# GREAT-WHU/DBA-Fusion

Hardware: AMD Instinct MI355X
Metric: DBA iterations/sec (25-KF, 96-edge, 512x512) [dba_update/s] (higher is better)
Workload: dtype f32 (BA, f64 reduced system) / f16 (correlation)

## Files before the change

dba-fusion_amd/csrc/ba_host.hip:

```cpp
#include <hip/hip_runtime.h>

#include <algorithm>
#include <atomic>
#include <cstdio>
#include <cstdlib>
#include <cstring>
#include <mutex>
#include <unordered_map>
#include <vector>

#include "ba_kernels.h"

#ifndef GRAM_F32_DEFAULT
#define GRAM_F32_DEFAULT true
#endif

namespace dba {

static thread_local char g_last_error[512] = "";

void set_last_error(const char *what, hipError_t e) {
  snprintf(g_last_error, sizeof(g_last_error), "%s -> %s", what, hipGetErrorString(e));
}

// ... 2 lines not shown
  static int num(const char *name) { const char *e = getenv(name); return e ? atoi(e) : 0; }
  static bool is(const char *name, const char *prefix) { const char *e = getenv(name); return e && !strncmp(e, prefix, strlen(prefix)); }
  int deterministic = is("DBA_DETERMINISTIC", "1");
  int solve_check = is("DBA_SOLVE_CHECK", "1");
  int schur_form = is("DBA_SCHUR_KERNEL", "r") ? 1 : (is("DBA_SCHUR_KERNEL", "f") || is("DBA_SCHUR_KERNEL", "g")) ? 2 : 0;
  int lin_ppl = num("DBA_LINEARIZE_PPL");
  bool lin_no_mfma = is("DBA_LINEARIZE_MFMA", "0");
  int lin_ew = num("DBA_LIN_EW");
  bool h_full = is("DBA_H_FULL", "1");
  int schur_nch = num("DBA_SCHUR_NCH");
  int gram_threads = num("DBA_SCHUR_WAVES") == 4 ? 256 : 512;
  bool gram_f32 = getenv("DBA_SCHUR_MFMA") ? is("DBA_SCHUR_MFMA", "f3") : GRAM_F32_DEFAULT;
  bool fuse_update = !is("DBA_BA_FUSE_UPDATE", "0");
  bool stage0_fold = getenv("DBA_BA_STAGE0") ? is("DBA_BA_STAGE0", "fold") : STAGE0_FOLD_DEFAULT;
  int schur_sparse_legacy = is("DBA_SCHUR_SPARSE", "legacy");
};
static const BaEnv &ba_env() { static const BaEnv env; return env; }

static std::atomic<int> g_schur_form{ba_env().schur_form};
static std::atomic<int> g_deterministic{ba_env().deterministic};
static std::atomic<int> g_solve_check{ba_env().solve_check};
static std::atomic<int> g_schur_sparse_legacy{ba_env().schur_sparse_legacy};

__global__ __launch_bounds__(256) void ba_solve_check_kernel(const double *__restrict__ H, const double *__restrict__ b, int n, double lm,
                                                             double ep, float *__restrict__ dx, int *__restrict__ meta) {
  __shared__ double s_res[256], s_mag[256];
  __shared__ int s_bad;
  if (meta[1] != 0) return;
  double res = 0.0, mag = 0.0;
  for (int i = threadIdx.x; i < n; i += blockDim.x) {
    double acc = -b[i], m = fabs(b[i]);
    for (int j = 0; j < n; j++) {
      double h = H[(size_t)max(i, j) * n + min(i, j)];
      if (i == j) h = fma(lm, h, h) + ep;
      const double t = h * (double)dx[j];
      acc += t, m += fabs(t);
    }
// ... 69 lines not shown
  L.E = take(sizeof(float) * (size_t)(P + N) * 6 * HW);
  L.Q = take(sizeof(float) * (size_t)Mmax * HW);
  L.w = take(sizeof(float) * (size_t)Mmax * HW);
  const size_t o_hparte = take(sizeof(float) * (size_t)(N > 0 ? N : 1) * nparts_max * HPE_STRIDE);
  const size_t o_aedge = take(sizeof(double) * 36 * (size_t)(N > 0 ? N : 1));
  L.dx = take(sizeof(float) * (size_t)(n6 > 0 ? n6 : 1));
  const size_t o_ptmp = take(sizeof(float) * 2 * 7 * (size_t)B);
  L.H = take(sizeof(double) * (size_t)(n6 > 0 ? n6 * (size_t)n6 : 1));
  L.b = take(sizeof(double) * (size_t)(n6 > 0 ? n6 : 1));
  size_t o_lscratch = 0;
  const bool lds_fits = ba_solve_fits_lds(n6);
  const bool want_scratch = !lds_fits || (ba_solve_band_supported(n6) && n6 >= 96);
  if (want_scratch) o_lscratch = take(sizeof(double) * ba_solve_scratch_doubles(n6));
  const size_t pairs_cap = (size_t)(P + N) * SCHUR_KP;
  const size_t o_pairs = take(sizeof(int) * 4 * (1 + pairs_cap));
  L.P = P;
  L.Mmax = Mmax;
  L.nchunks = nchunks;
  plan->layout = L;
  plan->bytes = off;
  plan->pairs_off = o_pairs, plan->pairs_cap = (int)pairs_cap;
  plan->P = P;
  plan->N = N;
  plan->B = B;
  plan->HW = HW;
  plan->nchunks = nchunks;
  plan->ht = ht, plan->wd = wd, plan->t0 = t0, plan->t1 = t1;
  if (ws) {
    if (ws_bytes < off) return DBA_ERR_WORKSPACE;
    char *base = static_cast<char *>(ws);
    plan->T.meta = reinterpret_cast<int *>(base + L.meta);
    plan->T.kx = reinterpret_cast<int *>(base + L.kx);
    plan->T.frame_slot = reinterpret_cast<int *>(base + o_fslot);
    plan->T.eoff = reinterpret_cast<int *>(base + o_eoff);
    plan->T.elist = reinterpret_cast<int *>(base + o_elist);
    plan->T.elist_rank = reinterpret_cast<int *>(base + o_erank);
    plan->T.fpose = reinterpret_cast<int *>(base + o_fpose);
    plan->T.einfo = reinterpret_cast<int *>(base + o_einfo);
    plan->T.rowinfo = reinterpret_cast<int *>(base + o_rowinfo);
    plan->T.fhead = reinterpret_cast<int *>(base + o_fhead);
    plan->T.frow = reinterpret_cast<int *>(base + o_frow);
    plan->T.gkey = reinterpret_cast<int *>(base + o_gkey);
    plan->T.pairs = reinterpret_cast<int *>(base + o_pairs);
    plan->T.pairs_cap = (int)pairs_cap;
    plan->T.Mmax = Mmax;
    plan->T.B = B;
    plan->W.E = reinterpret_cast<float *>(base + L.E);
    plan->W.Q = reinterpret_cast<float *>(base + L.Q);
    plan->W.w = reinterpret_cast<float *>(base + L.w);
    plan->W.HpartE = reinterpret_cast<float *>(base + o_hparte);
    plan->W.Aedge = reinterpret_cast<double *>(base + o_aedge);
    plan->W.dx = reinterpret_cast<float *>(base + L.dx);
    plan->W.poses_tmp = reinterpret_cast<float *>(base + o_ptmp);
    plan->W.H = reinterpret_cast<double *>(base + L.H);
    plan->W.b = reinterpret_cast<double *>(base + L.b);
    plan->W.Lscratch = want_scratch ? reinterpret_cast<double *>(base + o_lscratch) : nullptr;
    plan->W.nparts = nparts;
    plan->W.ppl = ppl;
  }
  return DBA_OK;
}

static int ba_prepare_stage(const BaPlan &plan, const int64_t *ii, const int64_t *jj, int eta_rows, int check, bool judge_band,
                            hipStream_t stream) {
  const int N = plan.N, B = plan.B, P = plan.P;
  if (N > 0 && (!ii || !jj)) return DBA_ERR_ARG;
  const int want = std::max(std::max(N, B), P);
  const int threads = std::min(1024, std::max(64, (want + 63) / 64 * 64));
  const size_t scan_ints = std::max<size_t>(std::max(threads, P), N > threads ? 1024 : 0) + 32;
  const size_t lds = sizeof(int) * ((size_t)B + 2 * (size_t)plan.T.Mmax + 1 + scan_ints + 2 * ((size_t)plan.T.Mmax + 1));
  if (lds > 160 * 1024 || P > 16384) return DBA_ERR_UNSUPPORTED;
  if (lds > 64 * 1024) {
    DBA_HIP_CHECK(hipFuncSetAttribute(reinterpret_cast<const void *>(&ba_prepare_kernel),
// ... 3 lines not shown
  int *band_verdict = max_nt ? solver_verdict_slot(plan.T.meta) : nullptr;
  hipLaunchKernelGGL(ba_prepare_kernel, dim3(1), dim3(threads), lds, stream, ii, jj, N, B, plan.t0, plan.t1,
                     (int)scan_ints, ba_schur_frame_form(N, P) ? 1 : 0, check ? 1 : 0, eta_rows,
                     eta_rows > 1 ? ws_eta_status(plan.T.meta) : nullptr, plan.T, band_verdict, max_nt);
  DBA_LAUNCH_CHECK();
  return DBA_OK;
}

static int ba_linearize_stage(const BaPlan &plan, const BaProblem &g, const float *poses, const float *disps, float alpha,
                              int upd, float *poses_out, float *disps_w, hipStream_t stream, const BaStage0 *s0 = nullptr) {
  if (!poses || !disps || !g.intrinsics || !g.disps_sens || !g.eta || g.eta_rows < 1) return DBA_ERR_ARG;
  if (g.eta_rows > 1 && g.eta_rows > plan.T.Mmax) return DBA_ERR_ARG;
  if (plan.N > 0 && (!g.targets || !g.weights || !g.jj)) return DBA_ERR_ARG;
  if (s0 && (upd != 0 || plan.W.ppl != 1)) return DBA_ERR_ARG;
  const BaStage0 none = {nullptr, 0, 0, nullptr, nullptr, 0};
#define LAUNCH_LIN_TF(PPL, MF, EW, TF)                                                                                        \
  hipLaunchKernelGGL((ba_linearize_kernel<PPL, MF, EW, TF>), dim3(plan.nchunks * EW, plan.T.Mmax + (TF ? 2 : 1)), dim3(256), 0, \
                     stream, poses, disps, g.intrinsics, g.disps_sens, g.targets, g.weights, g.eta, g.eta_rows, g.jj,         \
                     g.frame_owned, plan.N, plan.HW, plan.wd, plan.t0, plan.P, alpha, upd, poses_out, disps_w, plan.T, plan.W, \
                     TF ? *s0 : none)
#define LAUNCH_LIN(PPL, MF, EW) do { if (s0) LAUNCH_LIN_TF(PPL, MF, EW, true); else LAUNCH_LIN_TF(PPL, MF, EW, false); } while (0)
  if (plan.W.ppl == 4) LAUNCH_LIN_TF(4, false, 1, false);
  else if (plan.W.ppl == 2) LAUNCH_LIN_TF(2, false, 1, false);
  else if (ba_env().lin_no_mfma) LAUNCH_LIN(1, false, 1);
  else {
    const int env_ew = ba_env().lin_ew;
    const long waves2 = (long)plan.nchunks * 2 * 4 * plan.T.Mmax;
    const bool one = env_ew ? env_ew == 1 : waves2 > 4096;
    if (one) LAUNCH_LIN(1, true, 1);
    else LAUNCH_LIN(1, true, 2);
  }
#undef LAUNCH_LIN
#undef LAUNCH_LIN_TF
  DBA_LAUNCH_CHECK();
// ... 2 lines not shown

static int ba_reduce_stage(const BaPlan &plan, const int64_t *ii, const int64_t *jj, const uint8_t *frame_owned, int motion_only,
                           int lower, hipStream_t stream) {
  const int N = plan.N;
  const int ablocks = (N + 3) / 4;
  if (plan.P <= 0) return DBA_OK;
  if (ba_env().h_full) lower = 0;
  const bool fixed = g_deterministic.load(std::memory_order_relaxed) != 0;
  if (fixed) lower |= 2;
  if (!motion_only) {
    if (!ba_schur_frame_form(N, plan.P)) {
      if (g_schur_sparse_legacy.load(std::memory_order_relaxed))
        hipLaunchKernelGGL(ba_schur_kernel, dim3(plan.P + N + ablocks, SCHUR_KP, SCHUR_CH), dim3(256), 0, stream, ii, jj,
                           frame_owned, N, plan.HW, plan.t0, plan.P, lower, plan.T, plan.W);
      else
        hipLaunchKernelGGL(ba_schur_pairs_kernel, dim3(ablocks + plan.pairs_cap * SCHUR_CH), dim3(256), 0, stream, ii, jj,
                           frame_owned, N, plan.HW, plan.t0, plan.P, lower, plan.T, plan.W);
    } else {
      const int px = 1024;
      int nch = ba_env().schur_nch > 0 ? ba_env().schur_nch : (plan.HW + px - 1) / px;
      nch = std::max(1, std::min(nch, (plan.HW + 15) / 16));
      const dim3 grid((unsigned)(plan.T.Mmax * nch + ablocks));
      const int gram_threads = ba_env().gram_threads;
      const bool f32 = ba_env().gram_f32;
#define GRAM_LAUNCH(V, F)                                                                                     \
  hipLaunchKernelGGL((ba_schur_gram_kernel<V, F>), grid, dim3(gram_threads), 0, stream, ii, jj, frame_owned, \
                     N, plan.HW, plan.t0, plan.P, nch, lower, plan.T, plan.W)
      if (plan.HW % 4 == 0) { if (f32) GRAM_LAUNCH(true, true); else GRAM_LAUNCH(true, false); }
      else { if (f32) GRAM_LAUNCH(false, true); else GRAM_LAUNCH(false, false); }
#undef GRAM_LAUNCH
    }
    DBA_LAUNCH_CHECK();
  } else if (ablocks > 0) {
    hipLaunchKernelGGL(ba_assemble_kernel, dim3(ablocks), dim3(256), 0, stream, ii, jj, frame_owned, N, plan.t0, plan.P,
                       lower, plan.T, plan.W);
    DBA_LAUNCH_CHECK();
  }
// ... 20 lines not shown
  DBA_LAUNCH_CHECK();
  return DBA_OK;
}

static int ba_solve_stage(const BaPlan &plan, float lm, float ep, const int *fpose, int hint, hipStream_t stream) {
  const int rc = launch_ba_solve(plan.W.H, plan.W.b, fpose, 6 * plan.P, (double)lm, (double)ep, plan.W.dx, plan.T.meta,
                                 plan.W.Lscratch, stream, nullptr, hint, (fpose && fpose == plan.T.fpose) ? plan.T.meta + 16 : nullptr);
  if (rc != DBA_OK) return rc;
  if (g_solve_check.load(std::memory_order_relaxed)) return ba_solve_check_launch(plan, lm, ep, stream);
  return DBA_OK;
}

static int ba_update_launch(const BaPlan &plan, float *poses, float *disps, const int64_t *jj, const uint8_t *frame_owned,
                            int update_poses, int update_disps, float *dz_out, float *dx_out, hipStream_t stream,
                            const float *poses_src = nullptr, float disp_floor = 0.f) {
  dim3 grid((plan.HW + 255) / 256, plan.T.Mmax + 1 + (disp_floor > 0.f ? plan.B : 0));
  hipLaunchKernelGGL(ba_update_kernel, grid, dim3(256), 0, stream, poses, poses_src, disps, jj, frame_owned, plan.HW, plan.t0,
                     plan.P, update_poses, update_disps, dz_out, dx_out, plan.T, plan.W, disp_floor);
  DBA_LAUNCH_CHECK();
  return DBA_OK;
}

static bool ba_stage0_folds(const BaPlan &plan, const BaProblem &g, const BaRun &run) {
  return ba_env().stage0_fold && run.prepared == 2 && run.iterations > 0 && !g.frame_owned && !run.exchange && !run.window_fpose &&
         plan.W.ppl == 1 && plan.N <= FOLD_MAX_N && plan.B <= FOLD_MAX_B && (plan.N == 0 || (g.ii && g.jj));
}

int ba_run_loop(const BaPlan &plan, const BaProblem &g, float *poses, float *disps, const BaRun &run, hipStream_t stream) {
  const int *fpose = run.window_fpose ? run.window_fpose : plan.T.fpose;
  int rc;
  const bool fold = ba_stage0_folds(plan, g, run);
// ... 137 lines not shown
  const int rc = ba_plan(N, B, ht, wd, t0, t1, nullptr, 0, &plan);
  if (rc != DBA_OK) return rc;
  *out = plan.layout;
  return DBA_OK;
}

int dba_ba_pairs_table(int N, int B, int ht, int wd, int t0, int t1, size_t *offset, int *capacity) {
  BaPlan plan;
  const int rc = ba_plan(N, B, ht, wd, t0, t1, nullptr, 0, &plan);
  if (rc != DBA_OK) return rc;
  if (offset) *offset = plan.pairs_off;
  if (capacity) *capacity = plan.pairs_cap;
  return DBA_OK;
}

int dba_ba_schur_sparse_select(int legacy) {
  if (legacy != 0 && legacy != 1) return DBA_ERR_ARG;
  g_schur_sparse_legacy.store(legacy, std::memory_order_relaxed);
  return DBA_OK;
}

int dba_ba_poll_eta_error(int *eta_rows, int *num_kx) { return ws_poll_eta(nullptr, eta_rows, num_kx); }

int dba_ba_poll_eta_error_ws(int N, int B, int ht, int wd, int t0, int t1, void *ws, size_t ws_bytes, int *eta_rows, int *num_kx) {
  DBA_PLAN_OR_RETURN(plan);
  return ws_poll_eta(plan.T.meta, eta_rows, num_kx);
}

int dba_ba_gather_edges(const float *target_inac, const float *weight_inac, const int64_t *ii_inac, const int64_t *jj_inac,
                        int n_inac, const int64_t *sel, int n_sel, const float *target_act, const float *weight_act,
// ... 307 lines not shown
```

dba-fusion_amd/csrc/ba_kernels.h:

```cpp
#pragma once
#include "common.h"

namespace dba {

constexpr int HPE_STRIDE = 32;
#ifndef SCHUR_KP_CFG
#define SCHUR_KP_CFG 8
#endif
#ifndef SCHUR_CH_CFG
#define SCHUR_CH_CFG 2
#endif
constexpr int SCHUR_KP = SCHUR_KP_CFG;
constexpr int SCHUR_CH = SCHUR_CH_CFG;

struct BaTables {
  int *meta;
  int *kx;
  int *frame_slot;
  int *eoff;
  int *elist;
  int *elist_rank;
  int *fpose;
  int *einfo;
  int *rowinfo;
  int *fhead;
  int *frow;
  int *gkey;
  int *pairs;
  int pairs_cap;
  int Mmax, B;
};

struct BaBuffers {
  float *E;
  float *Q;
  float *w;
  float *HpartE;
  double *Aedge;
  double *H;
  double *b;
  float *dx;
  double *Lscratch;
  float *poses_tmp;
  int nparts;
  int ppl;
};

struct BaPlan {
  BaTables T;
  BaBuffers W;
  dba_ba_layout layout;
  size_t bytes;
  size_t pairs_off;
  int pairs_cap;
  int P, N, B, HW, nchunks;
  int ht, wd, t0, t1;
};

int ba_plan(int N, int B, int ht, int wd, int t0, int t1, void *ws, size_t ws_bytes, BaPlan *plan);
#define DBA_PLAN_OR_RETURN(plan) \
  BaPlan plan;                   \
  if (const int plan_rc_ = ::dba::ba_plan(N, B, ht, wd, t0, t1, ws, ws_bytes, &plan)) return plan_rc_

constexpr int GKEY_MAGIC = 0x6b657935;
__global__ void ba_prepare_kernel(const int64_t *ii, const int64_t *jj, int N, int B, int t0, int t1, int scan_ints,
                                  int ftable, int check, int eta_rows, int *status, BaTables T, int *band_verdict, int max_nt);
bool ba_schur_frame_form(int N, int P);
struct BaStage0 {
// ... 3 lines not shown
  int max_nt;
};
constexpr int FOLD_MAX_N = 256, FOLD_MAX_B = 512;
constexpr int FOLD_SCAN_INTS = FOLD_MAX_B + 32;
template <int PPL, bool MF, int EW, bool TF>
__global__ void ba_linearize_kernel(const float *poses, const float *disps, const float *intrinsics,
                                    const float *disps_sens, const float *targets, const float *weights,
                                    const float *eta, int eta_rows, const int64_t *jj,
                                    const uint8_t *frame_owned, int N, int HW, int wd, int t0, int P,
                                    float alpha, int upd, float *poses_out, float *disps_w, BaTables T, BaBuffers W,
                                    BaStage0 S0);
__global__ void ba_assemble_kernel(const int64_t *ii, const int64_t *jj, const uint8_t *frame_owned, int N,
                                   int t0, int P, int lower, BaTables T, BaBuffers W);
__global__ void ba_schur_kernel(const int64_t *ii, const int64_t *jj, const uint8_t *frame_owned, int N, int HW,
                                int t0, int P, int lower, BaTables T, BaBuffers W);
__global__ void ba_schur_pairs_kernel(const int64_t *ii, const int64_t *jj, const uint8_t *frame_owned, int N, int HW,
                                      int t0, int P, int lower, BaTables T, BaBuffers W);
__global__ void ba_symmetrize_kernel(double *H, int n);
struct ExportArg {
  double A[36];
};
__global__ void ba_export_kernel(const double *H, const double *b, int n, double *out, int gtsam, ExportArg arg, double stab,
                                 unsigned *counter, int *host_flag, int seq);
__global__ void ba_fixed_to_f64_kernel(double *H, double *b, int n);
constexpr int GRAM_LIST_CAP = 1024;
template <bool VEC, bool F32>
__global__ void ba_schur_gram_kernel(const int64_t *ii, const int64_t *jj, const uint8_t *frame_owned, int N, int HW,
                                     int t0, int P, int nch, int lower, BaTables T, BaBuffers W);
__global__ void ba_update_kernel(float *poses, const float *poses_src, float *disps, const int64_t *jj, const uint8_t *frame_owned,
                                 int HW, int t0, int P, int update_poses, int update_disps, float *dz_out,
// ... 52 lines not shown
```

dba-fusion_amd/csrc/ba_kernels.hip:

```cpp
#include "ba_kernels.h"
#include "ba_solve_admit.h"

#include <cstdio>
#include <cstring>

namespace dba {

__device__ __forceinline__ int wave_incl_scan(int v, int lane) {
#pragma unroll
  for (int off = 1; off < 64; off <<= 1) {
    const int o = __shfl_up(v, off, 64);
    if (lane >= off) v += o;
  }
  return v;
}

__device__ void ba_prepare_body(int *sm, const int64_t *__restrict__ ii, const int64_t *__restrict__ jj, int N, int B, int t0,
                                int t1, int scan_ints, int ftable, int check, int eta_rows, int *__restrict__ status,
                                const BaTables &T, int *__restrict__ band_verdict, int max_nt) {
  int *flag = sm;
  int *cnt = sm + B;
  int *kxs = cnt + T.Mmax + 1;
  int *scan = kxs + T.Mmax;
  int *vcnt = scan + scan_ints;
// ... 127 lines not shown
          const int x = sii[q];
          const bool same = ((x & (VBIT - 1)) == f);
          rank += same;
          vrank += same ? (x >> 30) : 0;
        }
        pos = cnt[m] + rank;
        T.elist[pos] = tid;
        if (myvalid) atomicAdd(&vcnt[m], 1);
      }
      emit_edge(tid, m, pos, my_j);
    }
    if (!ftable) {
      for (int m = tid; m < T.Mmax; m += nt) T.fhead[4 * m] = -1, T.fhead[4 * m + 2] = 0;
      __syncthreads();
      if (wave == 0) {
        int carry = 0;
        for (int base = 0; base <= T.Mmax; base += 64) {
          const int m = base + lane;
          const int v = (m < T.Mmax) ? vcnt[m] : 0;
          const int pc = v * (v + 1) / 2;
          const int w = wave_incl_scan(pc, lane);
          if (m <= T.Mmax) poff[m] = carry + w - pc;
          carry += __shfl(w, 63, 64);
        }
      }
      __syncthreads();
      const int npairs = poff[T.Mmax];
      const bool listed = npairs <= T.pairs_cap;
      int4 *pl = reinterpret_cast<int4 *>(T.pairs) + 1;
      if (tid == 0) *reinterpret_cast<int4 *>(T.pairs) = make_int4(listed ? npairs : -1, 0, 0, 0);
      if (listed && myvalid) {
        const int m = slot_of(my_i), v = vcnt[m], pp = kxs[m] - t0, tg = my_j - t0;
        const int vr = ((pp >= 0 && pp < P) ? 1 : 0) + vrank;
        int o = poff[m] + vr * v - vr * (vr - 1) / 2;
        pl[o++] = make_int4(P + tid, P + tid, tg | (tg << 16), m);
        const int f = my_i & (VBIT - 1);
        for (int q = tid + 1; q < N; q++)
          if (sii[q] == (f | VBIT)) pl[o++] = make_int4(P + tid, P + q, tg | (((int)jj[q] - t0) << 16), m);
      }
// ... 364 lines not shown
    const float *__restrict__ weights, const float *__restrict__ eta, int eta_rows,
    const int64_t *__restrict__ jj, const uint8_t *__restrict__ frame_owned, int N, int HW, int wd,
    int t0, int P, float alpha, int upd_arg, float *__restrict__ poses_out, float *__restrict__ disps_w, BaTables T,
    BaBuffers W, BaStage0 S0) {
  const int upd = TF ? 0 : (T.gkey[7] ? 0 : upd_arg);
#ifdef LIN_PROF
  unsigned long long lp_ = wall_clock64();
  const unsigned long long lp_start_ = lp_;
#endif
  constexpr int EB = 16;
  __shared__ float s_pose[EB][12];
  __shared__ __attribute__((aligned(16))) float s_adj[EB][28];
  __shared__ int s_edge[EB][2];
  constexpr int RED_FLOATS = MF ? MFS_FLOATS : 64 * RED_PITCH;
  __shared__ __attribute__((aligned(16))) float s_red[4][RED_FLOATS];
  const int m = blockIdx.y;
  if constexpr (TF) {
    if (m == T.Mmax + 1) {
      static_assert(!TF || 5 * FOLD_MAX_B + 3 + FOLD_SCAN_INTS <= 4 * RED_FLOATS, "stage 0 does not fit the staging tiles");
      if (blockIdx.x == 0)
        ba_prepare_body(reinterpret_cast<int *>(&s_red[0][0]), S0.ii, jj, N, T.B, t0, S0.t1, FOLD_SCAN_INTS, S0.ftable, 1, eta_rows,
                        S0.status, T, S0.band_verdict, S0.max_nt);
      return;
    }
  }
  if (m == T.Mmax) {
    const int n6 = 6 * P;
    const size_t total = (size_t)n6 * n6;
    for (size_t i = (size_t)blockIdx.x * blockDim.x + threadIdx.x; i < total; i += (size_t)gridDim.x * blockDim.x)
      W.H[i] = 0.0;
    if (blockIdx.x == 0) {
      for (int i = threadIdx.x; i < n6; i += blockDim.x) W.b[i] = 0.0;
      if (upd && poses_out)
        for (int f = threadIdx.x; f < T.B; f += blockDim.x) {
          float pr[7];
          load_pose(poses, W.dx, f, t0, P, true, pr);
#pragma unroll
          for (int c = 0; c < 7; c++) poses_out[7 * f + c] = pr[c];
        }
    }
    return;
  }
  int frame, e0 = 0, e1 = 0;
  __shared__ int2 s_out[TF ? FOLD_MAX_N : 1];
  if constexpr (TF) {
    __shared__ unsigned s_fmask[FOLD_MAX_B / 32];
// ... 31 lines not shown
    for (int w = 0; w < 4; w++) {
      const int c = s_wcnt[w];
      before += (w < (tid >> 6)) ? c : 0;
      e1 += c;
    }
    if (mine) s_out[before + __popcll(bal & ((1ull << (tid & 63)) - 1ull))] = make_int2(tid, my_j);
  } else {
    const int M = T.meta[0];
    if (m >= M) return;
    frame = T.kx[m];
    if (frame_owned && !frame_owned[frame]) return;
  }

  const int lane = lane_id();
  const int wv = threadIdx.x >> 6, ew = wv % EW;
  const int wave_global = blockIdx.x * (4 / EW) + wv / EW;
  const int kbase = wave_global * (WAVE * PPL) + lane;
  const int nparts = W.nparts;

  float intr[4] = {intrinsics[0], intrinsics[1], intrinsics[2], intrinsics[3]};
  int kc[PPL];
  bool active[PPL];
  float u[PPL], v[PPL], disp[PPL];
#pragma unroll
  for (int q = 0; q < PPL; q++) {
    const int k = kbase + WAVE * q;
    active[q] = k < HW;
    kc[q] = active[q] ? k : 0;
    u[q] = (float)(kc[q] % wd);
    v[q] = (float)(kc[q] / wd);
    disp[q] = disps[(size_t)frame * HW + kc[q]];
// ... 24 lines not shown
  for (int batch = e0; batch < e1; batch += EB) {
    const int cnt = min(EB, e1 - batch);
    __syncthreads();
    LP(1);
    if ((int)threadIdx.x < cnt) {
      const int2 ei = TF ? s_out[batch + threadIdx.x] : *reinterpret_cast<const int2 *>(T.einfo + 2 * (batch + threadIdx.x));
      const int n = ei.x, jx = ei.y;
      double t64[3], R64[9];
      edge_pose64(poses, W.dx, frame, jx, t0, P, upd != 0, t64, R64);
      s_edge[threadIdx.x][0] = n;
      s_edge[threadIdx.x][1] = jx;
#pragma unroll
      for (int c = 0; c < 3; c++) s_pose[threadIdx.x][c] = (float)t64[c];
#pragma unroll
      for (int c = 0; c < 9; c++) s_pose[threadIdx.x][3 + c] = (float)R64[c];
      double *Aw = (blockIdx.x == 0) ? W.Aedge + (size_t)n * 36 : nullptr;
      float *As = s_adj[threadIdx.x];
#pragma unroll
      for (int k = 0; k < 3; k++) {
#pragma unroll
        for (int c = 0; c < 3; c++) {
          const double rkc = -R64[3 * k + c];
          const int k1 = (k + 1) % 3, k2 = (k + 2) % 3;
          const double x = t64[k2] * R64[3 * k1 + c] - t64[k1] * R64[3 * k2 + c];
          As[6 * k + c] = (float)rkc, As[6 * k + 3 + c] = (float)x, As[18 + 3 * k + c] = (float)rkc;
          if (Aw) Aw[6 * k + c] = rkc, Aw[6 * k + 3 + c] = x, Aw[6 * (3 + k) + c] = 0.0, Aw[6 * (3 + k) + 3 + c] = rkc;
        }
      }
    }
    __syncthreads();
    LP(2);
// ... 547 lines not shown
}

__global__ __launch_bounds__(256) void ba_schur_pairs_kernel(const int64_t *__restrict__ ii,
                                                             const int64_t *__restrict__ jj,
                                                             const uint8_t *__restrict__ frame_owned, int N, int HW,
                                                             int t0, int P, int lower, BaTables T, BaBuffers W) {
  __shared__ float red[4][44];
  const int ablk = (N + 3) / 4;
  if ((int)blockIdx.x < ablk) {
    ba_assemble_block((int)blockIdx.x, ii, jj, frame_owned, N, t0, P, lower, T, W);
    return;
  }
  const int wg = (int)blockIdx.x - ablk;
  const int np = T.pairs[0];
  if (np < 0) {
    schur_rows_body(red, wg / (SCHUR_KP * SCHUR_CH), (wg / SCHUR_CH) % SCHUR_KP, SCHUR_KP, wg % SCHUR_CH, SCHUR_CH, frame_owned,
                    HW, t0, P, lower, T, W);
    return;
  }
  const int pi = wg / SCHUR_CH, ch = wg % SCHUR_CH;
  if (pi >= np) return;
  const int4 pr = reinterpret_cast<const int4 *>(T.pairs)[1 + pi];
  const int r1 = pr.x, r2 = pr.y, tgt1 = pr.z & 0xffff, tgt2 = pr.z >> 16, m = pr.w;
  if (frame_owned && !frame_owned[T.kx[m]]) return;
  const int chunk = (HW + SCHUR_CH - 1) / SCHUR_CH;
  const int k0 = ch * chunk, k1 = min(HW, k0 + chunk);
  const bool batch = chunk <= 256 * SCHUR_BATCH;
  const float *E1 = W.E + (size_t)r1 * 6 * HW;
  const float *E2 = W.E + (size_t)r2 * 6 * HW;
  const float *Qm = W.Q + (size_t)m * HW;
  const float *wm = W.w + (size_t)m * HW;
  const int n6 = 6 * P;
  if (r1 != r2) schur_pair_block<false, false>(red, batch, E1, E2, Qm, wm, HW, k0, k1, tgt1, tgt2, n6, lower, W);
  else if (lower & 1) schur_pair_block<true, true>(red, batch, E1, E2, Qm, wm, HW, k0, k1, tgt1, tgt2, n6, lower, W);
  else schur_pair_block<true, false>(red, batch, E1, E2, Qm, wm, HW, k0, k1, tgt1, tgt2, n6, lower, W);
}

constexpr int GRAM_MAX_T = 5;
constexpr int GRAM_MAX_ROWS = (16 * GRAM_MAX_T - 1) / 6;
constexpr int GRAM_MAX_TILES = GRAM_MAX_T * (GRAM_MAX_T + 1) / 2;
typedef double gram_d4 __attribute__((ext_vector_type(4)));

template <int T>
struct GramStage {
  lin_f4 q;
  lin_f4 e[T];
};

template <int T, bool VEC>
__device__ __forceinline__ void gram_load(GramStage<T> &S, const float *const (&bp)[T], const float *qm, int g, int gend,
// ... 187 lines not shown
  }
}

template <bool VEC, bool F32>
__global__ __launch_bounds__(512, 2) void ba_schur_gram_kernel(const int64_t *__restrict__ ii, const int64_t *__restrict__ jj,
                                                               const uint8_t *__restrict__ frame_owned, int N, int HW,
                                                               int t0, int P, int nch, int lower, BaTables T, BaBuffers W) {
  __shared__ double red[GRAM_MAX_TILES * 256];
  __shared__ int s_tgt[64];
  const int tid = threadIdx.x, lane = tid & 63;
  const int ablk = (N + 3) / 4;
  if ((int)blockIdx.x < ablk) {
    if (tid < 256) ba_assemble_block((int)blockIdx.x, ii, jj, frame_owned, N, t0, P, lower, T, W);
    return;
  }
  const int fblk = (int)blockIdx.x - ablk;
  const int m = fblk / nch, ch = fblk - m * nch;
  const int4 fh = *reinterpret_cast<const int4 *>(T.fhead + 4 * m);
  const int frame = fh.x, nrows = fh.z;
  if (frame < 0 || nrows == 0) return;
  if (frame_owned && !frame_owned[frame]) return;
  const int cpx = ((HW + nch - 1) / nch + 15) / 16 * 16;
  const int c0 = ch * cpx, c1 = min(HW, c0 + cpx);
  if (c0 >= c1) return;
  const float *wm = W.w + (size_t)m * HW, *qm = W.Q + (size_t)m * HW;
  const int n6 = 6 * P;
  const int *frow = T.frow + 2 * fh.y;
  if (nrows > GRAM_MAX_ROWS) {
    gram_frame_pairs(W, wm, qm, frow, nrows, c0, c1, HW, n6, (lower & 1) != 0, (lower & 2) != 0, reinterpret_cast<float *>(red));
    return;
  }
  int my_row = 0, my_tgt = 0;
// ... 108 lines not shown
      *counter = 0;
      __threadfence_system();
      __hip_atomic_store(host_flag, seq, __ATOMIC_RELEASE, __HIP_MEMORY_SCOPE_SYSTEM);
    }
  }
}

__global__ __launch_bounds__(256) void ba_update_kernel(float *__restrict__ poses, const float *__restrict__ poses_src,
                                                        float *__restrict__ disps,
                                                        const int64_t *__restrict__ jj,
                                                        const uint8_t *__restrict__ frame_owned, int HW,
                                                        int t0, int P, int update_poses, int update_disps,
                                                        float *__restrict__ dz_out,
                                                        float *__restrict__ dx_out, BaTables T, BaBuffers W,
                                                        float disp_floor) {
  const int m = blockIdx.y;
  if (T.gkey[7]) {
    if (m == T.Mmax && blockIdx.x == 0 && dx_out)
      for (int i = threadIdx.x; i < 6 * P; i += blockDim.x) dx_out[i] = 0.f;
    const int k = blockIdx.x * blockDim.x + threadIdx.x;
    if (m < T.Mmax && k < HW && dz_out && update_disps) dz_out[(size_t)m * HW + k] = 0.f;
    return;
  }
  if (m > T.Mmax) {
    const int frame = m - T.Mmax - 1;
    const int slot = T.frame_slot[frame];
    if (update_disps && slot >= 0 && slot < T.meta[0] && (!frame_owned || frame_owned[frame])) return;
    const int k = blockIdx.x * blockDim.x + threadIdx.x;
    if (k >= HW) return;
    const size_t fk = (size_t)frame * HW + k;
    if (disps[fk] < disp_floor) disps[fk] = disp_floor;
    return;
  }
  if (m == T.Mmax) {
    if (blockIdx.x != 0) return;
    if (dx_out)
      for (int i = threadIdx.x; i < 6 * P; i += blockDim.x) dx_out[i] = W.dx[i];
    if (!update_poses) return;
    for (int p = threadIdx.x; p < P; p += blockDim.x) {
      float pr[7];
      load_pose(poses_src ? poses_src : poses, W.dx, t0 + p, t0, P, true, pr);
#pragma unroll
      for (int c = 0; c < 7; c++) poses[7 * (t0 + p) + c] = pr[c];
    }
    return;
  }
  if (!update_disps) return;
  const int M = T.meta[0];
  if (m >= M) return;
  const int frame = T.kx[m];
  if (frame_owned && !frame_owned[frame]) return;
  const int k = blockIdx.x * blockDim.x + threadIdx.x;
  if (k >= HW) return;

  const float dz = backsub_pixel(T, W, m, frame, k, HW, t0, P);
  const size_t mk = (size_t)m * HW + k;
  const size_t fk = (size_t)frame * HW + k;
  float d = disps[fk] + dz;
  if (disp_floor > 0.f) d = (d < disp_floor) ? disp_floor : d;
  disps[fk] = d;
  if (dz_out) dz_out[mk] = dz;
}

__global__ __launch_bounds__(256) void ba_gather_edges_kernel(const float2 *__restrict__ tgt_inac, const float2 *__restrict__ wgt_inac,
                                                              const int64_t *__restrict__ ii_inac, const int64_t *__restrict__ jj_inac,
                                                              const int64_t *__restrict__ sel, int n_sel, int n_inac,
                                                              const float2 *__restrict__ tgt_act, const float2 *__restrict__ wgt_act,
// ... 29 lines not shown
```

dba-fusion_amd/dbaf_amd/_lib.py:

```python
import ctypes
import os
import weakref

import torch

_HERE = os.path.dirname(os.path.abspath(__file__))
LIB_PATH = os.environ.get("DBA_HIP_LIB") or os.path.join(os.path.dirname(_HERE), "lib", "libdba_hip.so")

DBA_F32, DBA_F16, DBA_F64, DBA_U8 = 0, 1, 2, 3
_ERR = {-1: "DBA_ERR_ARG", -2: "DBA_ERR_WORKSPACE", -3: "DBA_ERR_HIP", -4: "DBA_ERR_UNSUPPORTED"}

c_int, c_float, c_size_t, c_void_p = ctypes.c_int, ctypes.c_float, ctypes.c_size_t, ctypes.c_void_p


class BaLayout(ctypes.Structure):
    _fields_ = [(n, c_size_t) for n in ("H", "b", "dx", "meta", "E", "Q", "w", "kx")] + \
               [("P", c_int), ("Mmax", c_int), ("nchunks", c_int)]


class ShardExchange(ctypes.Structure):
    _fields_ = [("world", c_int), ("rank", c_int), ("comm", c_void_p), ("peer_regions", c_void_p),
                ("peer_epoch", ctypes.POINTER(ctypes.c_uint)), ("peer_max_doubles", c_size_t), ("peer_status", c_void_p),
                ("band_idx", c_void_p), ("band_len", c_size_t), ("band_buf", c_void_p),
                ("my_rows", c_void_p), ("n_mine", c_int), ("kmax", c_int), ("all_rows", c_void_p), ("all_slots", c_void_p),
# ... 40 lines not shown
    "dba_ba_prepare_keyed": (c_int, [_P, _P] + [c_int] * 8 + [_P, c_size_t, _P]),
    "dba_ba_workspace_init": (c_int, [c_int] * 6 + [_P, c_size_t, _P]),
    "dba_ba_solver_verdict": (c_int, [c_int] * 6 + [_P, c_size_t]),
    "dba_ba_poll_eta_error": (c_int, [ctypes.POINTER(c_int), ctypes.POINTER(c_int)]),
    "dba_ba_poll_eta_error_ws": (c_int, [c_int] * 6 + [_P, c_size_t, ctypes.POINTER(c_int), ctypes.POINTER(c_int)]),
    "dba_ba_gather_edges": (c_int, [_P] * 4 + [c_int, _P, c_int] + [_P] * 4 + [c_int] * 3 + [_P] * 5),
    "dba_ba_linearize": (c_int, [_P] * 7 + [c_int] + [_P] * 3 + [c_int] * 6 + [c_float, _P, c_size_t, _P]),
    "dba_ba_reduce": (c_int, [_P] * 3 + [c_int] * 7 + [_P, c_size_t, _P]),
    "dba_ba_schur_select": (c_int, [c_int]),
    "dba_ba_schur_select_thread": (c_int, [c_int]),
    "dba_ba_schur_auto_form": (c_int, [c_int, c_int]),
    "dba_ba_schur_thread_form": (c_int, []),
    "dba_ba_schur_generation": (c_int, []),
    "dba_ba_schur_sparse_select": (c_int, [c_int]),
    "dba_ba_pairs_table": (c_int, [c_int] * 6 + [ctypes.POINTER(c_size_t), ctypes.POINTER(c_int)]),
    "dba_ba_set_deterministic": (c_int, [c_int]),
    "dba_ba_set_solve_check": (c_int, [c_int]),
    "dba_ba_solve_check": (c_int, [c_int] * 6 + [c_float, c_float, _P, c_size_t, _P]),
    "dba_ba_symmetrize": (c_int, [c_int] * 6 + [_P, c_size_t, _P]),
    "dba_ba_solve": (c_int, [c_int] * 6 + [c_float, c_float, _P, c_size_t, _P]),
    "dba_ba_solve_skyline": (c_int, [c_int] * 6 + [c_float, c_float, _P, _P, c_size_t, _P]),
    "dba_ba_update": (c_int, [_P] * 5 + [c_int] * 8 + [_P, _P, c_size_t, _P]),
    "dba_ba_shard_front": (c_int, [_P] * 7 + [c_int] + [_P] * 3 + [c_int] * 6 + [c_float, c_int, _P, c_size_t, _P]),
    "dba_ba_shard_back": (c_int, [_P] * 5 + [c_int] * 6 + [c_float, c_float, c_int, _P, c_int, _P, c_size_t, _P]),
    "dba_comm_unique_id": (c_int, [_P]),
    "dba_comm_create": (c_int, [_P, c_int, c_int, ctypes.POINTER(_P)]),
    "dba_comm_destroy": (c_int, [_P]),
    "dba_comm_info": (c_int, [_P, ctypes.POINTER(c_int), ctypes.POINTER(c_int)]),
    "dba_comm_allreduce_f64": (c_int, [_P, c_size_t, _P]),
    "dba_ba_sharded_run": (c_int, [_P] * 7 + [c_int] + [_P] * 3 + [c_int] * 7 + [c_float, c_float, c_float, c_int, _P, c_int,
# ... 229 lines not shown
```

include/dba_hip.h:

```cpp
#ifndef DBA_HIP_H
#define DBA_HIP_H

#include <stddef.h>
#include <stdint.h>

#ifdef __cplusplus
extern "C" {
#endif

enum {
  DBA_OK = 0,
  DBA_ERR_ARG = -1,
  DBA_ERR_WORKSPACE = -2,
  DBA_ERR_HIP = -3,
  DBA_ERR_UNSUPPORTED = -4
};

enum { DBA_F32 = 0, DBA_F16 = 1, DBA_F64 = 2, DBA_U8 = 3 };

typedef void *dba_stream_t;

const char *dba_version(void);
const char *dba_last_error(void);

// ... 25 lines not shown
                     const float *eta, int eta_rows, const int64_t *ii, const int64_t *jj,
                     const uint8_t *frame_owned, int N, int B, int ht, int wd, int t0, int t1,
                     float alpha, void *ws, size_t ws_bytes, dba_stream_t stream);

int dba_ba_reduce(const int64_t *ii, const int64_t *jj, const uint8_t *frame_owned, int N, int B,
                  int ht, int wd, int t0, int t1, int motion_only, void *ws, size_t ws_bytes,
                  dba_stream_t stream);

int dba_ba_schur_select(int form);
int dba_ba_schur_select_thread(int form);
int dba_ba_schur_thread_form(void);
int dba_ba_schur_auto_form(int N, int P);
int dba_ba_schur_generation(void);
int dba_ba_schur_sparse_select(int legacy);
int dba_ba_pairs_table(int N, int B, int ht, int wd, int t0, int t1, size_t *offset, int *capacity);

int dba_ba_set_deterministic(int on);

int dba_ba_set_solve_check(int on);
int dba_ba_solve_check(int N, int B, int ht, int wd, int t0, int t1, float lm, float ep, void *ws, size_t ws_bytes,
                       dba_stream_t stream);

int dba_ba_symmetrize(int N, int B, int ht, int wd, int t0, int t1, void *ws, size_t ws_bytes, dba_stream_t stream);

int dba_ba_solve(int N, int B, int ht, int wd, int t0, int t1, float lm, float ep, void *ws,
                 size_t ws_bytes, dba_stream_t stream);
int dba_ba_solve_skyline(int N, int B, int ht, int wd, int t0, int t1, float lm, float ep, const int32_t *fpose, void *ws,
                         size_t ws_bytes, dba_stream_t stream);

int dba_ba_update(float *poses, float *disps, const int64_t *ii, const int64_t *jj,
// ... 464 lines not shown
```

Measured before the change: 4124.

## Place BA linearize and Schur pair blocks on XCDs by frame for L2 locality

Adds an XCD-aware block-id remapping so that every workgroup touching a given frame (linearize) or a given frame's pair group (Schur pairs) lands on the same XCD, since consecutive block ids round-robin across the MI355X's 8 XCDs. The prepare kernel now orders the pair prefix-scan by XCD group and records per-XCD group offsets, and the Schur pairs kernel loops over several pairs per block within its XCD group. The aim is better reuse of per-frame E/Q/w data in each XCD's private L2. The cost is possible load imbalance across XCDs, extra serialized work per block, padded grids, and reliance on an assumed round-robin dispatch order. Gram and update placement are added but off by default.

```diff
diff --git a/dba-fusion_amd/csrc/ba_host.hip b/dba-fusion_amd/csrc/ba_host.hip
--- a/dba-fusion_amd/csrc/ba_host.hip
+++ b/dba-fusion_amd/csrc/ba_host.hip
@@ -40,6 +40,7 @@
   bool fuse_update = !is("DBA_BA_FUSE_UPDATE", "0");
   bool stage0_fold = getenv("DBA_BA_STAGE0") ? is("DBA_BA_STAGE0", "fold") : STAGE0_FOLD_DEFAULT;
   int schur_sparse_legacy = is("DBA_SCHUR_SPARSE", "legacy");
+  int xcd = getenv("DBA_BA_XCD") ? (num("DBA_BA_XCD") & BA_XCD_ALL) : BA_XCD_DEFAULT;
 };
 static const BaEnv &ba_env() { static const BaEnv env; return env; }
 
@@ -47,6 +48,7 @@
 static std::atomic<int> g_deterministic{ba_env().deterministic};
 static std::atomic<int> g_solve_check{ba_env().solve_check};
 static std::atomic<int> g_schur_sparse_legacy{ba_env().schur_sparse_legacy};
+static std::atomic<int> g_xcd{ba_env().xcd};
 
 __global__ __launch_bounds__(256) void ba_solve_check_kernel(const double *__restrict__ H, const double *__restrict__ b, int n, double lm,
                                                              double ep, float *__restrict__ dx, int *__restrict__ meta) {
@@ -146,12 +148,13 @@
   if (want_scratch) o_lscratch = take(sizeof(double) * ba_solve_scratch_doubles(n6));
   const size_t pairs_cap = (size_t)(P + N) * SCHUR_KP;
   const size_t o_pairs = take(sizeof(int) * 4 * (1 + pairs_cap));
+  const size_t o_pgrp = take(sizeof(int) * (BA_NUM_XCD + 1));
   L.P = P;
   L.Mmax = Mmax;
   L.nchunks = nchunks;
   plan->layout = L;
   plan->bytes = off;
-  plan->pairs_off = o_pairs, plan->pairs_cap = (int)pairs_cap;
+  plan->pairs_off = o_pairs, plan->pairs_cap = (int)pairs_cap, plan->pgrp_off = o_pgrp;
   plan->P = P;
   plan->N = N;
   plan->B = B;
@@ -175,6 +178,7 @@
     plan->T.gkey = reinterpret_cast<int *>(base + o_gkey);
     plan->T.pairs = reinterpret_cast<int *>(base + o_pairs);
     plan->T.pairs_cap = (int)pairs_cap;
+    plan->T.pgrp = reinterpret_cast<int *>(base + o_pgrp);
     plan->T.Mmax = Mmax;
     plan->T.B = B;
     plan->W.E = reinterpret_cast<float *>(base + L.E);
@@ -189,6 +193,7 @@
     plan->W.Lscratch = want_scratch ? reinterpret_cast<double *>(base + o_lscratch) : nullptr;
     plan->W.nparts = nparts;
     plan->W.ppl = ppl;
+    plan->W.xcd = g_xcd.load(std::memory_order_relaxed);
   }
   return DBA_OK;
 }
@@ -222,10 +227,17 @@
   if (plan.N > 0 && (!g.targets || !g.weights || !g.jj)) return DBA_ERR_ARG;
   if (s0 && (upd != 0 || plan.W.ppl != 1)) return DBA_ERR_ARG;
   const BaStage0 none = {nullptr, 0, 0, nullptr, nullptr, 0};
+  BaBuffers Wl = plan.W;
+  const bool placed = (plan.W.xcd & ((upd & 2) ? BA_XCD_LIN : BA_XCD_LIN_FIRST)) != 0;
+  Wl.xcd = placed ? (Wl.xcd | BA_XCD_LIN) : (Wl.xcd & ~BA_XCD_LIN);
+  auto lin_grid = [&](int chunks, int rows_behind) {
+    return placed ? dim3((unsigned)(ba_xcd_frame_ids(plan.T.Mmax, chunks) + rows_behind * chunks))
+                                     : dim3((unsigned)chunks, (unsigned)(plan.T.Mmax + rows_behind));
+  };
 #define LAUNCH_LIN_TF(PPL, MF, EW, TF)                                                                                        \
-  hipLaunchKernelGGL((ba_linearize_kernel<PPL, MF, EW, TF>), dim3(plan.nchunks * EW, plan.T.Mmax + (TF ? 2 : 1)), dim3(256), 0, \
+  hipLaunchKernelGGL((ba_linearize_kernel<PPL, MF, EW, TF>), lin_grid(plan.nchunks * EW, TF ? 2 : 1), dim3(256), 0,             \
                      stream, poses, disps, g.intrinsics, g.disps_sens, g.targets, g.weights, g.eta, g.eta_rows, g.jj,         \
-                     g.frame_owned, plan.N, plan.HW, plan.wd, plan.t0, plan.P, alpha, upd, poses_out, disps_w, plan.T, plan.W, \
+                     g.frame_owned, plan.N, plan.HW, plan.wd, plan.t0, plan.P, alpha, upd, poses_out, disps_w, plan.T, Wl,     \
                      TF ? *s0 : none)
 #define LAUNCH_LIN(PPL, MF, EW) do { if (s0) LAUNCH_LIN_TF(PPL, MF, EW, true); else LAUNCH_LIN_TF(PPL, MF, EW, false); } while (0)
   if (plan.W.ppl == 4) LAUNCH_LIN_TF(4, false, 1, false);
@@ -258,13 +270,16 @@
         hipLaunchKernelGGL(ba_schur_kernel, dim3(plan.P + N + ablocks, SCHUR_KP, SCHUR_CH), dim3(256), 0, stream, ii, jj,
                            frame_owned, N, plan.HW, plan.t0, plan.P, lower, plan.T, plan.W);
       else
-        hipLaunchKernelGGL(ba_schur_pairs_kernel, dim3(ablocks + plan.pairs_cap * SCHUR_CH), dim3(256), 0, stream, ii, jj,
-                           frame_owned, N, plan.HW, plan.t0, plan.P, lower, plan.T, plan.W);
+        hipLaunchKernelGGL(ba_schur_pairs_kernel,
+                           dim3((plan.W.xcd & BA_XCD_SCHUR) ? ba_schur_pairs_xcd_grid(N, plan.pairs_cap).ids()
+                                                            : ablocks + plan.pairs_cap * SCHUR_CH),
+                           dim3(256), 0, stream, ii, jj, frame_owned, N, plan.HW, plan.t0, plan.P, lower, plan.T, plan.W);
     } else {
       const int px = 1024;
       int nch = ba_env().schur_nch > 0 ? ba_env().schur_nch : (plan.HW + px - 1) / px;
       nch = std::max(1, std::min(nch, (plan.HW + 15) / 16));
-      const dim3 grid((unsigned)(plan.T.Mmax * nch + ablocks));
+      const dim3 grid((plan.W.xcd & BA_XCD_GRAM) ? (unsigned)(ba_xcd_round_up(ablocks) + ba_xcd_frame_ids(plan.T.Mmax, nch))
+                                                  : (unsigned)(plan.T.Mmax * nch + ablocks));
       const int gram_threads = ba_env().gram_threads;
       const bool f32 = ba_env().gram_f32;
 #define GRAM_LAUNCH(V, F)                                                                                     \
@@ -315,7 +330,9 @@
 static int ba_update_launch(const BaPlan &plan, float *poses, float *disps, const int64_t *jj, const uint8_t *frame_owned,
                             int update_poses, int update_disps, float *dz_out, float *dx_out, hipStream_t stream,
                             const float *poses_src = nullptr, float disp_floor = 0.f) {
-  dim3 grid((plan.HW + 255) / 256, plan.T.Mmax + 1 + (disp_floor > 0.f ? plan.B : 0));
+  const int chunks = (plan.HW + 255) / 256, rows_behind = 1 + (disp_floor > 0.f ? plan.B : 0);
+  dim3 grid(chunks, plan.T.Mmax + rows_behind);
+  if (plan.W.xcd & BA_XCD_UPDATE) grid = dim3((unsigned)(ba_xcd_frame_ids(plan.T.Mmax, chunks) + rows_behind * chunks));
   hipLaunchKernelGGL(ba_update_kernel, grid, dim3(256), 0, stream, poses, poses_src, disps, jj, frame_owned, plan.HW, plan.t0,
                      plan.P, update_poses, update_disps, dz_out, dx_out, plan.T, plan.W, disp_floor);
   DBA_LAUNCH_CHECK();
@@ -483,6 +500,37 @@
   return DBA_OK;
 }
 
+int dba_ba_xcd_select(int mask) {
+  if (mask < -1 || mask > BA_XCD_ALL) return DBA_ERR_ARG;
+  g_xcd.store(mask < 0 ? ba_env().xcd : mask, std::memory_order_relaxed);
+  return DBA_OK;
+}
+
+int dba_ba_xcd_mask(void) { return g_xcd.load(std::memory_order_relaxed); }
+
+int dba_ba_xcd_frame_ids(int F, int C) { return (F < 0 || C <= 0) ? DBA_ERR_ARG : ba_xcd_frame_ids(F, C); }
+
+int dba_ba_xcd_frame_item(int id, int base, int F, int C, int *item, int *row) {
+  if (F < 0 || C <= 0 || base % BA_NUM_XCD || !item || !row) return DBA_ERR_ARG;
+  return ba_xcd_frame_item(id, base, F, C, *item, *row) ? 1 : 0;
+}
+
+int dba_ba_xcd_group_item(int id, int base, int S, const int32_t *goff, int CH, int k, int *entry, int *chunk) {
+  if (S < 0 || CH <= 0 || k < 0 || base % BA_NUM_XCD || !goff || !entry || !chunk) return DBA_ERR_ARG;
+  return ba_xcd_group_item(id, base, S, goff, CH, k, *entry, *chunk) ? 1 : 0;
+}
+
+int dba_ba_xcd_pairs_grid(int N, int B, int ht, int wd, int t0, int t1, int *base, int *slots, size_t *pgrp_offset) {
+  BaPlan plan;
+  const int rc = ba_plan(N, B, ht, wd, t0, t1, nullptr, 0, &plan);
+  if (rc != DBA_OK) return rc;
+  const BaPairsXcdGrid grid = ba_schur_pairs_xcd_grid(N, plan.pairs_cap);
+  if (base) *base = grid.base;
+  if (slots) *slots = grid.S;
+  if (pgrp_offset) *pgrp_offset = plan.pgrp_off;
+  return DBA_OK;
+}
+
 int dba_ba_schur_sparse_select(int legacy) {
   if (legacy != 0 && legacy != 1) return DBA_ERR_ARG;
   g_schur_sparse_legacy.store(legacy, std::memory_order_relaxed);
diff --git a/dba-fusion_amd/csrc/ba_kernels.h b/dba-fusion_amd/csrc/ba_kernels.h
--- a/dba-fusion_amd/csrc/ba_kernels.h
+++ b/dba-fusion_amd/csrc/ba_kernels.h
@@ -1,5 +1,6 @@
 #pragma once
 #include "common.h"
+#include "ba_xcd.h"
 
 namespace dba {
 
@@ -28,6 +29,7 @@
   int *gkey;
   int *pairs;
   int pairs_cap;
+  int *pgrp;
   int Mmax, B;
 };
 
@@ -44,6 +46,7 @@
   float *poses_tmp;
   int nparts;
   int ppl;
+  int xcd;
 };
 
 struct BaPlan {
@@ -52,6 +55,7 @@
   dba_ba_layout layout;
   size_t bytes;
   size_t pairs_off;
+  size_t pgrp_off;
   int pairs_cap;
   int P, N, B, HW, nchunks;
   int ht, wd, t0, t1;
@@ -85,6 +89,13 @@
                                    int t0, int P, int lower, BaTables T, BaBuffers W);
 __global__ void ba_schur_kernel(const int64_t *ii, const int64_t *jj, const uint8_t *frame_owned, int N, int HW,
                                 int t0, int P, int lower, BaTables T, BaBuffers W);
+struct BaPairsXcdGrid {
+  int base, S;
+  int ids() const { return base + BA_NUM_XCD * S; }
+};
+inline BaPairsXcdGrid ba_schur_pairs_xcd_grid(int N, int pairs_cap) {
+  return {ba_xcd_round_up((N + 3) / 4), (pairs_cap * SCHUR_CH + BA_NUM_XCD - 1) / BA_NUM_XCD};
+}
 __global__ void ba_schur_pairs_kernel(const int64_t *ii, const int64_t *jj, const uint8_t *frame_owned, int N, int HW,
                                       int t0, int P, int lower, BaTables T, BaBuffers W);
 __global__ void ba_symmetrize_kernel(double *H, int n);
diff --git a/dba-fusion_amd/csrc/ba_kernels.hip b/dba-fusion_amd/csrc/ba_kernels.hip
--- a/dba-fusion_amd/csrc/ba_kernels.hip
+++ b/dba-fusion_amd/csrc/ba_kernels.hip
@@ -165,15 +165,21 @@
       for (int m = tid; m < T.Mmax; m += nt) T.fhead[4 * m] = -1, T.fhead[4 * m + 2] = 0;
       __syncthreads();
       if (wave == 0) {
+        const int G = (T.Mmax + BA_NUM_XCD - 1) / BA_NUM_XCD;
         int carry = 0;
-        for (int base = 0; base <= T.Mmax; base += 64) {
-          const int m = base + lane;
-          const int v = (m < T.Mmax) ? vcnt[m] : 0;
+        for (int base = 0; base < BA_NUM_XCD * G; base += 64) {
+          const int j = base + lane;
+          const int x = j / G, m = x + BA_NUM_XCD * (j - x * G);
+          const bool real = j < BA_NUM_XCD * G && m < T.Mmax;
+          const int v = real ? vcnt[m] : 0;
           const int pc = v * (v + 1) / 2;
           const int w = wave_incl_scan(pc, lane);
-          if (m <= T.Mmax) poff[m] = carry + w - pc;
+          if (real) poff[m] = carry + w - pc;
+          if (j < BA_NUM_XCD * G && j == x * G) T.pgrp[x] = carry + w - pc;
           carry += __shfl(w, 63, 64);
         }
+        if (lane == 0) poff[T.Mmax] = carry, T.pgrp[BA_NUM_XCD] = carry;
+        if (G == 0 && lane < BA_NUM_XCD) T.pgrp[lane] = 0;
       }
       __syncthreads();
       const int npairs = poff[T.Mmax];
@@ -568,11 +574,15 @@
   __shared__ int s_edge[EB][2];
   constexpr int RED_FLOATS = MF ? MFS_FLOATS : 64 * RED_PITCH;
   __shared__ __attribute__((aligned(16))) float s_red[4][RED_FLOATS];
-  const int m = blockIdx.y;
+  int bx = blockIdx.x, m = blockIdx.y, gx = gridDim.x;
+  if (W.xcd & BA_XCD_LIN) {
+    gx = (W.nparts / 4) * EW;
+    if (!ba_xcd_frame_item((int)blockIdx.x, 0, T.Mmax, gx, bx, m)) return;
+  }
   if constexpr (TF) {
     if (m == T.Mmax + 1) {
       static_assert(!TF || 5 * FOLD_MAX_B + 3 + FOLD_SCAN_INTS <= 4 * RED_FLOATS, "stage 0 does not fit the staging tiles");
-      if (blockIdx.x == 0)
+      if (bx == 0)
         ba_prepare_body(reinterpret_cast<int *>(&s_red[0][0]), S0.ii, jj, N, T.B, t0, S0.t1, FOLD_SCAN_INTS, S0.ftable, 1, eta_rows,
                         S0.status, T, S0.band_verdict, S0.max_nt);
       return;
@@ -581,9 +591,9 @@
   if (m == T.Mmax) {
     const int n6 = 6 * P;
     const size_t total = (size_t)n6 * n6;
-    for (size_t i = (size_t)blockIdx.x * blockDim.x + threadIdx.x; i < total; i += (size_t)gridDim.x * blockDim.x)
+    for (size_t i = (size_t)bx * blockDim.x + threadIdx.x; i < total; i += (size_t)gx * blockDim.x)
       W.H[i] = 0.0;
-    if (blockIdx.x == 0) {
+    if (bx == 0) {
       for (int i = threadIdx.x; i < n6; i += blockDim.x) W.b[i] = 0.0;
       if (upd && poses_out)
         for (int f = threadIdx.x; f < T.B; f += blockDim.x) {
@@ -645,7 +655,7 @@
 
   const int lane = lane_id();
   const int wv = threadIdx.x >> 6, ew = wv % EW;
-  const int wave_global = blockIdx.x * (4 / EW) + wv / EW;
+  const int wave_global = bx * (4 / EW) + wv / EW;
   const int kbase = wave_global * (WAVE * PPL) + lane;
   const int nparts = W.nparts;
 
@@ -700,7 +710,7 @@
       for (int c = 0; c < 3; c++) s_pose[threadIdx.x][c] = (float)t64[c];
 #pragma unroll
       for (int c = 0; c < 9; c++) s_pose[threadIdx.x][3 + c] = (float)R64[c];
-      double *Aw = (blockIdx.x == 0) ? W.Aedge + (size_t)n * 36 : nullptr;
+      double *Aw = (bx == 0) ? W.Aedge + (size_t)n * 36 : nullptr;
       float *As = s_adj[threadIdx.x];
 #pragma unroll
       for (int k = 0; k < 3; k++) {
@@ -1278,26 +1288,37 @@
   const int wg = (int)blockIdx.x - ablk;
   const int np = T.pairs[0];
   if (np < 0) {
+    if (wg >= T.pairs_cap * SCHUR_CH) return;
     schur_rows_body(red, wg / (SCHUR_KP * SCHUR_CH), (wg / SCHUR_CH) % SCHUR_KP, SCHUR_KP, wg % SCHUR_CH, SCHUR_CH, frame_owned,
                     HW, t0, P, lower, T, W);
     return;
   }
-  const int pi = wg / SCHUR_CH, ch = wg % SCHUR_CH;
-  if (pi >= np) return;
-  const int4 pr = reinterpret_cast<const int4 *>(T.pairs)[1 + pi];
-  const int r1 = pr.x, r2 = pr.y, tgt1 = pr.z & 0xffff, tgt2 = pr.z >> 16, m = pr.w;
-  if (frame_owned && !frame_owned[T.kx[m]]) return;
   const int chunk = (HW + SCHUR_CH - 1) / SCHUR_CH;
-  const int k0 = ch * chunk, k1 = min(HW, k0 + chunk);
   const bool batch = chunk <= 256 * SCHUR_BATCH;
-  const float *E1 = W.E + (size_t)r1 * 6 * HW;
-  const float *E2 = W.E + (size_t)r2 * 6 * HW;
-  const float *Qm = W.Q + (size_t)m * HW;
-  const float *wm = W.w + (size_t)m * HW;
   const int n6 = 6 * P;
-  if (r1 != r2) schur_pair_block<false, false>(red, batch, E1, E2, Qm, wm, HW, k0, k1, tgt1, tgt2, n6, lower, W);
-  else if (lower & 1) schur_pair_block<true, true>(red, batch, E1, E2, Qm, wm, HW, k0, k1, tgt1, tgt2, n6, lower, W);
-  else schur_pair_block<true, false>(red, batch, E1, E2, Qm, wm, HW, k0, k1, tgt1, tgt2, n6, lower, W);
+  auto run_pair = [&](int pi, int ch) {
+    const int4 pr = reinterpret_cast<const int4 *>(T.pairs)[1 + pi];
+    const int r1 = pr.x, r2 = pr.y, tgt1 = pr.z & 0xffff, tgt2 = pr.z >> 16, m = pr.w;
+    if (frame_owned && !frame_owned[T.kx[m]]) return;
+    const int k0 = ch * chunk, k1 = min(HW, k0 + chunk);
+    const float *E1 = W.E + (size_t)r1 * 6 * HW;
+    const float *E2 = W.E + (size_t)r2 * 6 * HW;
+    const float *Qm = W.Q + (size_t)m * HW;
+    const float *wm = W.w + (size_t)m * HW;
+    if (r1 != r2) schur_pair_block<false, false>(red, batch, E1, E2, Qm, wm, HW, k0, k1, tgt1, tgt2, n6, lower, W);
+    else if (lower & 1) schur_pair_block<true, true>(red, batch, E1, E2, Qm, wm, HW, k0, k1, tgt1, tgt2, n6, lower, W);
+    else schur_pair_block<true, false>(red, batch, E1, E2, Qm, wm, HW, k0, k1, tgt1, tgt2, n6, lower, W);
+  };
+  if (W.xcd & BA_XCD_SCHUR) {
+    const int base = ba_xcd_round_up(ablk), S = ((int)gridDim.x - base) / BA_NUM_XCD;
+    int pi, ch;
+    for (int k = 0; ba_xcd_group_item((int)blockIdx.x, base, S, T.pgrp, SCHUR_CH, k, pi, ch); k++) {
+      if (k) __syncthreads();
+      run_pair(pi, ch);
+    }
+    return;
+  }
+  if (wg / SCHUR_CH < np) run_pair(wg / SCHUR_CH, wg % SCHUR_CH);
 }
 
 constexpr int GRAM_MAX_T = 5;
@@ -1515,8 +1536,13 @@
     if (tid < 256) ba_assemble_block((int)blockIdx.x, ii, jj, frame_owned, N, t0, P, lower, T, W);
     return;
   }
-  const int fblk = (int)blockIdx.x - ablk;
-  const int m = fblk / nch, ch = fblk - m * nch;
+  int m, ch;
+  if (W.xcd & BA_XCD_GRAM) {
+    if (!ba_xcd_frame_item((int)blockIdx.x, ba_xcd_round_up(ablk), T.Mmax, nch, ch, m)) return;
+  } else {
+    const int fblk = (int)blockIdx.x - ablk;
+    m = fblk / nch, ch = fblk - m * nch;
+  }
   const int4 fh = *reinterpret_cast<const int4 *>(T.fhead + 4 * m);
   const int frame = fh.x, nrows = fh.z;
   if (frame < 0 || nrows == 0) return;
@@ -1655,11 +1681,14 @@
                                                         float *__restrict__ dz_out,
                                                         float *__restrict__ dx_out, BaTables T, BaBuffers W,
                                                         float disp_floor) {
-  const int m = blockIdx.y;
+  int bx = blockIdx.x, m = blockIdx.y;
+  if (W.xcd & BA_XCD_UPDATE) {
+    if (!ba_xcd_frame_item((int)blockIdx.x, 0, T.Mmax, (HW + 255) / 256, bx, m)) return;
+  }
   if (T.gkey[7]) {
-    if (m == T.Mmax && blockIdx.x == 0 && dx_out)
+    if (m == T.Mmax && bx == 0 && dx_out)
       for (int i = threadIdx.x; i < 6 * P; i += blockDim.x) dx_out[i] = 0.f;
-    const int k = blockIdx.x * blockDim.x + threadIdx.x;
+    const int k = bx * blockDim.x + threadIdx.x;
     if (m < T.Mmax && k < HW && dz_out && update_disps) dz_out[(size_t)m * HW + k] = 0.f;
     return;
   }
@@ -1667,14 +1696,14 @@
     const int frame = m - T.Mmax - 1;
     const int slot = T.frame_slot[frame];
     if (update_disps && slot >= 0 && slot < T.meta[0] && (!frame_owned || frame_owned[frame])) return;
-    const int k = blockIdx.x * blockDim.x + threadIdx.x;
+    const int k = bx * blockDim.x + threadIdx.x;
     if (k >= HW) return;
     const size_t fk = (size_t)frame * HW + k;
     if (disps[fk] < disp_floor) disps[fk] = disp_floor;
     return;
   }
   if (m == T.Mmax) {
-    if (blockIdx.x != 0) return;
+    if (bx != 0) return;
     if (dx_out)
       for (int i = threadIdx.x; i < 6 * P; i += blockDim.x) dx_out[i] = W.dx[i];
     if (!update_poses) return;
@@ -1691,7 +1720,7 @@
   if (m >= M) return;
   const int frame = T.kx[m];
   if (frame_owned && !frame_owned[frame]) return;
-  const int k = blockIdx.x * blockDim.x + threadIdx.x;
+  const int k = bx * blockDim.x + threadIdx.x;
   if (k >= HW) return;
 
   const float dz = backsub_pixel(T, W, m, frame, k, HW, t0, P);
diff --git a/dba-fusion_amd/csrc/ba_xcd.h b/dba-fusion_amd/csrc/ba_xcd.h
--- /dev/null
+++ b/dba-fusion_amd/csrc/ba_xcd.h
@@ -0,0 +1,37 @@
+#pragma once
+#include <hip/hip_runtime.h>
+
+namespace dba {
+
+constexpr int BA_NUM_XCD = 8;
+constexpr int BA_XCD_LIN = 1, BA_XCD_SCHUR = 2, BA_XCD_UPDATE = 4, BA_XCD_GRAM = 8, BA_XCD_LIN_FIRST = 16, BA_XCD_ALL = 31;
+#ifndef BA_XCD_DEFAULT
+#define BA_XCD_DEFAULT (BA_XCD_LIN | BA_XCD_SCHUR)
+#endif
+
+__host__ __device__ inline int ba_xcd_round_up(int n) { return (n + BA_NUM_XCD - 1) / BA_NUM_XCD * BA_NUM_XCD; }
+
+__host__ __device__ inline int ba_xcd_frame_ids(int F, int C) { return ba_xcd_round_up(F) * C; }
+__host__ __device__ inline bool ba_xcd_frame_item(int id, int base, int F, int C, int &c, int &row) {
+  const int rel = id - base, placed = ba_xcd_frame_ids(F, C);
+  if (rel < 0) return false;
+  if (rel >= placed) {
+    const int e = rel - placed;
+    row = F + e / C, c = e % C;
+    return true;
+  }
+  const int s = rel >> 3;
+  row = (id & (BA_NUM_XCD - 1)) + BA_NUM_XCD * (s / C), c = s % C;
+  return row < F;
+}
+
+__host__ __device__ inline bool ba_xcd_group_item(int id, int base, int S, const int *goff, int CH, int k, int &entry, int &chunk) {
+  const int rel = id - base;
+  if (rel < 0 || rel >= BA_NUM_XCD * S) return false;
+  const int x = id & (BA_NUM_XCD - 1), t = (rel >> 3) + k * S;
+  if (t >= (goff[x + 1] - goff[x]) * CH) return false;
+  entry = goff[x] + t / CH, chunk = t % CH;
+  return true;
+}
+
+}
diff --git a/dba-fusion_amd/dbaf_amd/_lib.py b/dba-fusion_amd/dbaf_amd/_lib.py
--- a/dba-fusion_amd/dbaf_amd/_lib.py
+++ b/dba-fusion_amd/dbaf_amd/_lib.py
@@ -78,6 +78,12 @@
     "dba_ba_schur_generation": (c_int, []),
     "dba_ba_schur_sparse_select": (c_int, [c_int]),
     "dba_ba_pairs_table": (c_int, [c_int] * 6 + [ctypes.POINTER(c_size_t), ctypes.POINTER(c_int)]),
+    "dba_ba_xcd_select": (c_int, [c_int]),
+    "dba_ba_xcd_mask": (c_int, []),
+    "dba_ba_xcd_frame_ids": (c_int, [c_int, c_int]),
+    "dba_ba_xcd_frame_item": (c_int, [c_int] * 4 + [ctypes.POINTER(c_int)] * 2),
+    "dba_ba_xcd_group_item": (c_int, [c_int] * 3 + [_P] + [c_int] * 2 + [ctypes.POINTER(c_int)] * 2),
+    "dba_ba_xcd_pairs_grid": (c_int, [c_int] * 6 + [ctypes.POINTER(c_int)] * 2 + [ctypes.POINTER(c_size_t)]),
     "dba_ba_set_deterministic": (c_int, [c_int]),
     "dba_ba_set_solve_check": (c_int, [c_int]),
     "dba_ba_solve_check": (c_int, [c_int] * 6 + [c_float, c_float, _P, c_size_t, _P]),
diff --git a/include/dba_hip.h b/include/dba_hip.h
--- a/include/dba_hip.h
+++ b/include/dba_hip.h
@@ -63,6 +63,12 @@
 int dba_ba_schur_generation(void);
 int dba_ba_schur_sparse_select(int legacy);
 int dba_ba_pairs_table(int N, int B, int ht, int wd, int t0, int t1, size_t *offset, int *capacity);
+int dba_ba_xcd_select(int mask);
+int dba_ba_xcd_mask(void);
+int dba_ba_xcd_frame_ids(int F, int C);
+int dba_ba_xcd_frame_item(int id, int base, int F, int C, int *item, int *row);
+int dba_ba_xcd_group_item(int id, int base, int S, const int32_t *goff, int CH, int k, int *entry, int *chunk);
+int dba_ba_xcd_pairs_grid(int N, int B, int ht, int wd, int t0, int t1, int *base, int *slots, size_t *pgrp_offset);
 
 int dba_ba_set_deterministic(int on);
 
```

After: 4199 (median of 4 runs). 1.02x the previous value.
